# sehyun03/MulActSeg

Hardware: AMD Instinct MI355X
Metric: superpixels scored/sec (higher is better)
Workload: dtype f32; 1 GPU; acquisition-round: PixBal+ban-ignore scorer on resident logits, Cityscapes pool shape [4,20,1024,2048] per step; per rank K single-pass scans (class prior + region sums + histograms) of its shard, then exchange 1 (all-gather class sums) + device class weights (k_class_weight) + weighted finalize + ban + exchange 2 (all-gather scores) + replicated K4 (keys, radix sort, fair-counting budget walk) ov; nseg=2048, id_dtype=int64, regions_scored=679936, budget_clicks=11159, regions_selected=6688

## Files before the change

include/mulactseg_hip.h:

```cpp
#ifndef MULACTSEG_HIP_H
#define MULACTSEG_HIP_H

#include <stddef.h>
#include <stdint.h>

#ifdef __cplusplus
extern "C" {
#endif

#define MAS_ID_I64 0
#define MAS_ID_I32 1
#define MAS_ID_U16 2
#define MAS_MAP_U8 3

#define MAS_MAX_CLASSES 32

#define MAS_SCORE_FRAC_BITS 40
#define MAS_PROB_FRAC_BITS 23
#define MAS_LOSS_FRAC_BITS 32

#define MAS_ABI_VERSION 9
int mas_abi_version(void);
const char* mas_error_string(int code);

// ... 44 lines not shown
int mas_partial_loss_bwd(const float* z, const void* spx, int spx_dtype, const uint8_t* mask, const uint32_t* bits,
                         const uint64_t* gmax, const float* scale ,
                         int N, int C, int H, int W, int S, float invT, int flags, float* dz, void* stream);

int mas_partial_loss_fwd_lowres(const float* zq, int h, int w, const void* spx, int spx_dtype, const uint8_t* mask,
                                const uint32_t* bits, int N, int C, int H, int W, int S, float invT, int flags,
                                uint64_t* gmax , uint64_t* acc , void* stream);
int mas_partial_loss_bwd_lowres(const float* zq, int h, int w, const void* spx, int spx_dtype, const uint8_t* mask,
                                const uint32_t* bits, const uint64_t* gmax, const float* scale , int N, int C, int H, int W,
                                int S, float invT, int flags, int64_t* dzq_fix , void* stream);
#define MAS_GRAD_FRAC_BITS 44
int mas_fix_to_float(const int64_t* fix, int64_t n, int frac_bits, float* out, void* stream);

size_t mas_partial_loss_work_bytes(int N, int S, int C, int flags);
int mas_partial_loss_fwd_fused(const float* z, int h, int w, const void* spx, int spx_dtype, const uint8_t* mask, const uint8_t* targets,
                               int cols_stored, int cols_used, const uint32_t* bits, int N, int C, int H, int W, int S, float invT, int flags,
                               const float* weights, void* work, size_t work_bytes, float* losses, void* stream);
int mas_partial_loss_bwd_fused(const float* z, int h, int w, const void* spx, int spx_dtype, const uint8_t* mask, const uint32_t* bits,
                               const void* work, const float* grad, const float* weights, int N, int C, int H, int W, int S, float invT,
                               int flags, float* dz, int64_t* dzq_fix, void* stream);


int mas_region_keys(const float* score, const uint8_t* valid, const int32_t* img_rank, int64_t n_img, int S,
                    uint64_t* keys , void* stream);

size_t mas_select_workspace_bytes(int64_t n);

int mas_sort_keys_desc(const uint64_t* keys_in, int64_t n, uint64_t* keys_out, void* workspace, size_t ws_bytes,
                       void* stream);

int mas_budget_walk(const uint64_t* sorted_keys, int64_t n, const uint8_t* region_cost, const int32_t* img_of_rank,
                    int S, int64_t budget, int64_t max_out, int64_t* n_selected,
                    int32_t* sel_img, int32_t* sel_id, float* sel_score, void* workspace, size_t ws_bytes, void* stream);

int mas_region_reweight(float* score, const int32_t* dominant, int64_t n, int ban_class, const float* cls_w ,
                        void* stream);

int mas_dominant_hist(const int32_t* dominant, int64_t n, int C, uint64_t* counts , void* stream);

int mas_minmax_normalize(float* scores, int64_t n, uint32_t* scratch2, void* stream);


#define MAS_LABELS_BAD_VALUE 1

int mas_region_label_counts(const void* spx, int spx_dtype, const uint8_t* labels, int H, int W, int nseg, int num_classes, int trim_k,
                            int32_t* full , int32_t* trimmed , int32_t* status ,
                            void* stream);

int mas_region_multi_hot(const int32_t* full, const int32_t* trimmed, const uint8_t* listed, int nseg, int num_classes,
                         uint8_t* bits , int64_t* size , void* stream);

int mas_region_dominant(const int32_t* full, const uint8_t* listed, const int32_t* drawn , int nseg, int num_classes,
                        int generate_ignore, int32_t* choice , void* stream);

int mas_region_paint(const void* spx, int spx_dtype, const uint8_t* labels, int H, int W, int nseg, const int32_t* choice,
                     int generate_ignore, uint8_t* out , void* stream);

int mas_spx_max_onehot(const void* target, int target_dtype, const void* spx, int spx_dtype, int H, int W, int nseg, int num_classes,
                       int32_t* seg_max , int32_t* status , uint8_t* mask ,
                       uint8_t* rows , void* stream);


int mas_iou_counts(const int64_t* outputs, const int64_t* outputs_all, const int64_t* targets, int64_t n,
                   int num_classes, int64_t ignore_label, uint64_t* counts , void* stream);

int mas_logits_iou_counts(const float* z, const int64_t* targets, int B, int channels, int H, int W, int num_classes,
// ... 180 lines not shown
```

mulactseg_amd/_lib.py:

```python
import ctypes
import os

_HERE = os.path.dirname(os.path.abspath(__file__))
LIB_PATH = os.environ.get("MAS_LIB") or os.path.join(_HERE, "libmulactseg_hip.so")

ID_I64, ID_I32, ID_U16 = 0, 1, 2
MAP_U8 = 3
MAX_CLASSES = 32
LABELS_BAD_VALUE = 1
SCORE_FRAC, PROB_FRAC, LOSS_FRAC = 40, 23, 32
LOSS_CE, LOSS_GROUP, LOSS_GROUP_ONLY_MULTI, LOSS_DECOMP, LOSS_TCE = 1, 2, 4, 8, 16
ACC_WORDS = 8
GRAD_FRAC = 44
MS_MAX_SOURCES = 16

SK_DMA, SK_NOSPLIT = 1, 2
LOWRES_GENERIC = 1
ABI_VERSION = 9

_c = ctypes
_vp, _i, _f, _i64, _d = _c.c_void_p, _c.c_int, _c.c_float, _c.c_int64, _c.c_double


class SkOpts(ctypes.Structure):
    _fields_ = [("flags", _c.c_uint), ("spin_limit", _c.c_uint), ("stamps", _c.c_void_p)]


SIGNATURES = {
    "mas_abi_version": (_i, []),
    "mas_error_string": (_c.c_char_p, [_i]),
    "mas_class_prob_sum": (_i, [_vp, _i, _i, _i, _i, _f, _vp, _vp]),
    "mas_bvsb_region_accum": (_i, [_vp, _vp, _i, _vp, _i, _i, _i, _i, _i, _f, _vp, _vp, _vp]),
    "mas_region_finalize": (_i, [_vp, _vp, _i64, _i, _i, _vp, _vp, _vp, _vp, _vp]),
    "mas_region_keys": (_i, [_vp, _vp, _vp, _i64, _i, _vp, _vp]),
    "mas_select_workspace_bytes": (_c.c_size_t, [_i64]),
    "mas_sort_keys_desc": (_i, [_vp, _i64, _vp, _vp, _c.c_size_t, _vp]),
    "mas_budget_walk": (_i, [_vp, _i64, _vp, _vp, _i, _i64, _i64, _vp, _vp, _vp, _vp, _vp, _c.c_size_t, _vp]),
    "mas_region_reweight": (_i, [_vp, _vp, _i64, _i, _vp, _vp]),
    "mas_dominant_hist": (_i, [_vp, _i64, _i, _vp, _vp]),
    "mas_minmax_normalize": (_i, [_vp, _i64, _vp, _vp]),
    "mas_region_label_counts": (_i, [_vp, _i, _vp, _i, _i, _i, _i, _i, _vp, _vp, _vp, _vp]),
    "mas_region_multi_hot": (_i, [_vp, _vp, _vp, _i, _i, _vp, _vp, _vp]),
    "mas_region_dominant": (_i, [_vp, _vp, _vp, _i, _i, _i, _vp, _vp]),
    "mas_region_paint": (_i, [_vp, _i, _vp, _i, _i, _i, _vp, _i, _vp, _vp]),
    "mas_spx_max_onehot": (_i, [_vp, _i, _vp, _i, _i, _i, _i, _i, _vp, _vp, _vp, _vp, _vp]),
    "mas_iou_counts": (_i, [_vp, _vp, _vp, _i64, _i, _i64, _vp, _vp]),
    "mas_logits_iou_counts": (_i, [_vp, _vp, _i, _i, _i, _i, _i, _i64, _vp, _vp]),
    "mas_lowres_iou_counts": (_i, [_vp, _vp, _i, _i, _i, _i, _i, _i, _i, _i64, _vp, _vp]),
    "mas_single_pass_accum": (_i, [_vp, _vp, _i, _i, _i, _i, _i, _i, _f, _vp, _vp, _vp, _vp]),
    "mas_single_pass_accum_lowres": (_i, [_vp, _i, _i, _vp, _i, _i, _i, _i, _i, _i, _f, _vp, _vp, _vp, _vp]),
    "mas_single_pass_accum_lowres_opt": (_i, [_vp, _i, _i, _vp, _i, _i, _i, _i, _i, _i, _f, _vp, _vp, _vp, _c.c_uint, _vp]),
    "mas_class_weight": (_i, [_vp, _i, _i, _i64, _i, _i, _d, _vp, _vp, _vp, _vp]),
    "mas_region_finalize_weighted": (_i, [_vp, _vp, _i64, _i, _vp, _i, _vp, _vp, _vp, _vp, _vp]),
    "mas_stage2_gather_protos": (_i, [_vp, _i, _i, _i, _i, _i, _vp, _i, _vp, _vp]),
    "mas_stage2_assign": (_i, [_vp, _i, _i, _i, _i, _i, _vp, _vp, _i, _vp, _vp, _vp, _vp, _vp]),
    "mas_stage2_adjacency": (_i, [_vp, _i, _i, _i, _vp, _vp, _vp]),
    "mas_stage2_propagate": (_i, [_vp, _i, _i, _i, _i, _i, _vp, _i, _vp, _vp, _vp, _vp, _vp, _vp, _vp, _vp]),
    "mas_aspp_dw3_fwd": (_i, [_vp, _vp, _vp, _vp, _i, _i, _i, _i, _i, _i, _i, _vp, _vp, _vp, _vp]),
    "mas_aspp_dw3_bwd_x": (_i, [_vp, _vp, _vp, _vp, _vp, _vp, _i, _i, _i, _i, _i, _i, _i, _vp, _vp]),
    "mas_aspp_dw3_bwd_w": (_i, [_vp, _vp, _vp, _vp, _i, _i, _i, _i, _i, _i, _i, _vp, _vp, _vp, _vp]),
    "mas_train_augment": (_i, [_vp, _i, _i, _i, _i, _vp, _vp, _i, _vp, _vp, _i, _vp, _vp, _i, _i, _i, _i, _i, _i, _i, _vp, _vp, _vp,
                               _vp, _i, _i64, _vp, _i, _vp, _i, _i64, _vp, _i, _vp, _vp]),
    "mas_upsample_bilinear_fwd": (_i, [_vp, _i64, _i, _i, _i, _i, _vp, _vp]),
    "mas_upsample_bilinear_bwd": (_i, [_vp, _i64, _i, _i, _i, _i, _vp, _vp]),
    "mas_ms_ensemble": (_i, [_vp, _vp, _vp, _i, _i, _i, _i, _i, _vp, _vp, _vp]),
    "mas_naive_plbl": (_i, [_vp, _i, _i, _i, _i, _i, _i, _vp, _f, _vp, _vp]),
    "mas_ms_naive_plbl": (_i, [_vp, _vp, _i, _i, _i, _i, _vp, _i, _i64, _vp, _vp, _vp]),
    "mas_render_labels": (_i, [_vp, _i, _i, _i, _i, _vp, _i, _i, _vp, _i, _vp, _vp, _vp]),
    "mas_render_lowres_pred": (_i, [_vp, _i, _i, _i, _i, _i, _i, _vp, _i, _vp, _vp, _vp]),
    "mas_bn_workspace_bytes": (_i64, [_i, _i, _i]),
# ... 121 lines not shown
```

mulactseg_amd/active_selection/engine.py:

```python
import numpy as np
import torch


class ShardPlan:

    def __init__(self, n_img, batch_size, rank=0, world=1):
        self.n_img, self.batch_size, self.rank, self.world = n_img, batch_size, rank, world
        self.n_batches = (n_img + batch_size - 1) // batch_size
        per = (self.n_batches + world - 1) // world
        self.batch_lo = min(rank * per, self.n_batches)
        self.batch_hi = min((rank + 1) * per, self.n_batches)
        self.img_lo = min(self.batch_lo * batch_size, n_img)
        self.img_hi = min(self.batch_hi * batch_size, n_img)
        self.per_rank_imgs = per * batch_size
        self.batch_of = (np.arange(n_img) // batch_size).astype(np.int32)

    @property
    def local_indices(self):
        return list(range(self.img_lo, self.img_hi))

    @property
    def n_local(self):
        return self.img_hi - self.img_lo

# ... 16 lines not shown
        return local
    pad = torch.zeros((plan.per_rank_imgs,) + tuple(local.shape[1:]), dtype=local.dtype, device=local.device)
    pad[:plan.n_local] = local
    out = torch.empty((plan.world * plan.per_rank_imgs,) + tuple(local.shape[1:]), dtype=local.dtype, device=local.device)
    d.all_gather_into_tensor(out, pad)
    return out[:plan.n_img].contiguous()


def class_weight_from_sums(prob_sum, hw, batch_of, n_batches, coeff):
    prob_sum = np.ascontiguousarray(prob_sum).view(np.uint64)
    n_img, C = prob_sum.shape
    batch_of = np.asarray(batch_of)
    sums = np.zeros((n_batches, C), dtype=np.uint64)
    np.add.at(sums, batch_of, prob_sum)
    n_in = np.bincount(batch_of, minlength=n_batches)[:n_batches]
    live = n_in > 0
    terms = (sums[live].astype(np.float64) / np.float64(8388608.0)) / (n_in[live].astype(np.float64) * np.float64(hw))[:, None]
    acc = np.cumsum(terms, axis=0)[-1] if terms.shape[0] else np.zeros(C, dtype=np.float64)
    cum = acc / np.float64(n_batches)
    t = np.float64(coeff) * cum + np.float64(1.0)
    return cum, (np.float64(1.0) / (t * t)).astype(np.float32)


class HipBackend:
    name = "hip"

    def __init__(self, device):
        from .. import _lib, ops
        self.device = torch.device(device)
        if self.device.type != 'cuda':
            raise _lib.MulActSegHipError("HipBackend needs a ROCm device, got %s (no CPU path exists)" % device)
        _lib.load()
        self.ops = ops

    def inv_temperature(self, T):
        return self.ops.inv_temperature(T)

    def class_prob_sum(self, logits, invT, out):
        self.ops.class_prob_sum(logits, invT, out=out)

    def region_accum(self, logits, spx, cls_w, S, invT, score_sum, hist):
        self.ops.bvsb_region_accum(logits, spx, cls_w, S, invT, score_sum=score_sum, hist=hist)

    def finalize(self, score_sum, hist, ban_class, want_hist_i64=False):
        return self.ops.region_finalize(score_sum, hist, ban_class, want_hist_i64)

    def single_pass(self, logits, spx, S, invT, prob_sum, class_sum, hist):
        self.ops.single_pass_accum(logits, spx, S, invT, prob_sum=prob_sum, class_sum=class_sum, hist=hist)

    def single_pass_lowres(self, zq, size, spx, S, invT, prob_sum, class_sum, hist):
        self.ops.single_pass_accum_lowres(zq, size, spx, S, invT, prob_sum=prob_sum, class_sum=class_sum, hist=hist)

    def class_weight(self, prob_sum, hw, batch_size, n_batches, coeff):
        cum, w, w31 = self.ops.class_weight(prob_sum.contiguous(), hw, batch_size, n_batches, coeff)
        w._mas_w31 = w31
        return cum, w

    def finalize_weighted(self, class_sum, hist, cls_w, ban_class, want_hist_i64=False):
        w31 = None if cls_w is None else getattr(cls_w, '_mas_w31', None)
        if w31 is None:
            w = torch.ones(hist.shape[-1], dtype=torch.float32, device=hist.device) if cls_w is None else cls_w.detach().to(hist.device)
            w31 = (w.double() * 2147483648.0).floor().to(torch.int64).view(torch.int32)[::2].contiguous()
        return self.ops.region_finalize_weighted(class_sum, hist, w31, ban_class, want_hist_i64)

    def minmax_normalize_(self, scores):
        return self.ops.minmax_normalize_(scores)

    def region_reweight_(self, scores, dominant, ban_class, cls_w):
        return self.ops.region_reweight_(scores, dominant, ban_class, cls_w)

    def dominant_hist(self, dominant, C):
        return self.ops.dominant_hist(dominant, C)

    def select(self, scores, valid, img_rank, img_of_rank, region_cost, budget, max_out):
        keys = self.ops.region_keys(scores, valid, img_rank)
        skeys = self.ops.sort_keys_desc(keys)
        nsel, simg, sid, ssc = self.ops.budget_walk(skeys, region_cost, img_of_rank, scores.shape[1], budget, max_out)
        n = int(nsel.item())
        return n, simg[:n].cpu().numpy(), sid[:n].cpu().numpy(), ssc[:n].cpu().numpy()

    def local_head(self, plan, scores, valid, img_rank, max_out):
        lo, hi = plan.img_lo, plan.img_hi
        head = torch.zeros(max_out, dtype=torch.int64, device=scores.device)
        if hi > lo:
            keys = self.ops.region_keys(scores[lo:hi].contiguous(), None if valid is None else valid[lo:hi].contiguous(),
                                        img_rank[lo:hi].contiguous())
            m = min(keys.numel(), max_out)
            head[:m] = self.ops.sort_keys_desc(keys)[:m]
        return head

    def walk_heads(self, heads, region_cost, img_of_rank, S, budget, max_out):
        nsel, simg, sid, ssc = self.ops.budget_walk(self.ops.sort_keys_desc(heads), region_cost, img_of_rank, S, budget, max_out)
        n = int(nsel.item())
        return n, simg[:n].cpu().numpy(), sid[:n].cpu().numpy(), ssc[:n].cpu().numpy()

    def select_sharded(self, plan, scores, valid, img_rank, img_of_rank, region_cost, budget, max_out):
        head = self.local_head(plan, scores, valid, img_rank, max_out)
        merged = torch.empty(plan.world * max_out, dtype=torch.int64, device=scores.device)
        _dist().all_gather_into_tensor(merged, head)
        return self.walk_heads(merged, region_cost, img_of_rank, scores.shape[1], budget, max_out)


def default_backend(device):
    return HipBackend(device)


def select_regions(backend, plan, scores, valid, img_rank, img_of_rank, region_cost, budget, max_out):
    if plan.world > 1 and max_out is not None and _dist() is not None and hasattr(backend, 'select_sharded'):
        return backend.select_sharded(plan, scores, valid, img_rank, img_of_rank, region_cost, budget, max_out)
    return backend.select(scores, valid, img_rank, img_of_rank, region_cost, budget, max_out)


class AcquisitionRound:

    def __init__(self, n_img, n_channels, n_superpixels, batch_size, temperature, backend, rank=None, world=None,
                 single_pass=False):
        r, w = current_rank_world()
        self.plan = ShardPlan(n_img, batch_size, r if rank is None else rank, w if world is None else world)
        self.C, self.S = n_channels, n_superpixels
        self.backend = backend
        self.invT = backend.inv_temperature(temperature)
        self.single_pass = single_pass
        dev = backend.device
        nl = max(self.plan.n_local, 1)
# ... 90 lines not shown
```

mulactseg_amd/csrc/select.hip:

```cpp
#include <cstring>

#include <rocprim/device/device_radix_sort.hpp>
#include <rocprim/device/device_scan.hpp>

#include "common.h"

namespace {

constexpr int kThreads = 256;

__device__ __forceinline__ unsigned order_bits(float f) {
    const unsigned b = mas_f2u(f);
    return (b & 0x80000000u) ? ~b : (b | 0x80000000u);
}
__device__ __forceinline__ float unorder_bits(unsigned o) {
    return mas_u2f((o & 0x80000000u) ? (o & 0x7fffffffu) : ~o);
}

inline int id_bits_for(int S) {
    int b = 1;
    while ((1LL << b) < S) ++b;
    return b;
}

// ... 90 lines not shown
    }
    __syncthreads();
    if ((int)threadIdx.x < C && s_cnt[threadIdx.x]) atomicAdd(&counts[threadIdx.x], (mas_u64)s_cnt[threadIdx.x]);
}

__global__ __launch_bounds__(kThreads) void k_minmax_nonzero(const float* __restrict__ u, long long n, unsigned* __restrict__ mm) {
    unsigned lo = 0xffffffffu, hi = 0u;
    for (long long i = (long long)blockIdx.x * kThreads + threadIdx.x; i < n; i += (long long)gridDim.x * kThreads) {
        const float v = u[i];
        const unsigned o = order_bits(v);
        if (v != 0.0f) lo = o < lo ? o : lo;
        hi = o > hi ? o : hi;
    }
#pragma unroll
    for (int off = MAS_WAVE / 2; off > 0; off >>= 1) {
        const unsigned l2 = __shfl_down(lo, off, MAS_WAVE), h2 = __shfl_down(hi, off, MAS_WAVE);
        lo = l2 < lo ? l2 : lo;
        hi = h2 > hi ? h2 : hi;
    }
    if ((threadIdx.x & (MAS_WAVE - 1)) == 0) {
        atomicMin(&mm[0], lo);
        atomicMax(&mm[1], hi);
    }
}

__global__ void k_minmax_init(unsigned* mm) { mm[0] = 0xffffffffu; mm[1] = 0u; }

__global__ __launch_bounds__(kThreads) void k_minmax_apply(float* __restrict__ u, long long n, const unsigned* __restrict__ mm) {
    const long long i = (long long)blockIdx.x * kThreads + threadIdx.x;
    if (i >= n) return;
    const float mn = unorder_bits(mm[0]);
    const float mx = unorder_bits(mm[1]) - mn;
    u[i] = (u[i] - mn) / mx;
}

inline size_t align_up(size_t v) { return (v + 255) & ~(size_t)255; }

size_t sort_temp_bytes(long long n) {
    size_t bytes = 0;
    mas_u64* nul = nullptr;
    (void)rocprim::radix_sort_keys_desc(nullptr, bytes, nul, nul, (size_t)n, 0, 64, (hipStream_t)0);
    return bytes;
}
size_t scan_temp_bytes(long long n) {
    size_t bytes = 0;
    unsigned* nul = nullptr;
    (void)rocprim::inclusive_scan(nullptr, bytes, nul, nul, (size_t)n, rocprim::plus<unsigned>(), (hipStream_t)0);
    return bytes;
}

}

extern "C" size_t mas_select_workspace_bytes(int64_t n) {
    if (n <= 0) return 0;
    const size_t t = sort_temp_bytes(n), u = scan_temp_bytes(n);
    return align_up(t > u ? t : u) + 2 * align_up(sizeof(unsigned) * (size_t)n) + 256;
}

extern "C" int mas_region_keys(const float* score, const uint8_t* valid, const int32_t* img_rank, int64_t n_img, int S,
                               uint64_t* keys, void* stream) {
    if (!score || !img_rank || !keys) return MAS_ERR_NULL;
    if (n_img <= 0 || S <= 0) return MAS_ERR_SHAPE;
    const int b = id_bits_for(S);
    if (b > 24 || n_img > (1LL << (32 - b))) return MAS_ERR_RANGE;
    const long long n = (long long)n_img * S;
    const long long nblk = (n + kThreads - 1) / kThreads;
// ... 15 lines not shown
    return e == hipSuccess ? mas_launch_status() : (int)e;
}

extern "C" int mas_budget_walk(const uint64_t* sorted_keys, int64_t n, const uint8_t* region_cost, const int32_t* img_of_rank,
                               int S, int64_t budget, int64_t max_out, int64_t* n_selected, int32_t* sel_img, int32_t* sel_id,
                               float* sel_score, void* workspace, size_t ws_bytes, void* stream) {
    if (!sorted_keys || !img_of_rank || !n_selected || !sel_img || !sel_id || !sel_score || !workspace) return MAS_ERR_NULL;
    if (n <= 0 || S <= 0 || max_out <= 0 || budget < 0) return MAS_ERR_SHAPE;
    if (n > (1LL << 24)) return MAS_ERR_RANGE;
    if (ws_bytes < mas_select_workspace_bytes(n)) return MAS_ERR_WORKSPACE;
    hipStream_t st = static_cast<hipStream_t>(stream);
    const int b = id_bits_for(S);
    unsigned char* ws = static_cast<unsigned char*>(workspace);
    size_t temp = scan_temp_bytes(n);
    const size_t t = sort_temp_bytes(n);
    const size_t temp_region = align_up(t > temp ? t : temp);
    unsigned* cost = reinterpret_cast<unsigned*>(ws + temp_region);
    unsigned* prefix = reinterpret_cast<unsigned*>(ws + temp_region + align_up(sizeof(unsigned) * (size_t)n));
    const mas_u64* keys = reinterpret_cast<const mas_u64*>(sorted_keys);
    unsigned long long* nsel = reinterpret_cast<unsigned long long*>(n_selected);
    const long long nblk = (n + kThreads - 1) / kThreads;
    hipLaunchKernelGGL(k_set_u64, dim3(1), dim3(1), 0, st, nsel, (unsigned long long)n);
    hipLaunchKernelGGL(k_walk_cost, dim3((unsigned)nblk), dim3(kThreads), 0, st, keys, (long long)n, region_cost, img_of_rank, S, b, cost);
    hipError_t e = rocprim::inclusive_scan(ws, temp, cost, prefix, (size_t)n, rocprim::plus<unsigned>(), st);
    if (e != hipSuccess) return (int)e;
    hipLaunchKernelGGL(k_walk_find, dim3((unsigned)nblk), dim3(kThreads), 0, st, keys, prefix, (long long)n,
                       (unsigned long long)budget, nsel);
    const long long oblk = (max_out + kThreads - 1) / kThreads;
    hipLaunchKernelGGL(k_walk_emit, dim3((unsigned)oblk), dim3(kThreads), 0, st, keys, nsel, (long long)max_out, img_of_rank, b,
                       sel_img, sel_id, sel_score);
    return mas_launch_status();
}

extern "C" int mas_minmax_normalize(float* scores, int64_t n, uint32_t* scratch2, void* stream) {
    if (!scores || !scratch2) return MAS_ERR_NULL;
    if (n <= 0) return MAS_ERR_SHAPE;
    hipStream_t st = static_cast<hipStream_t>(stream);
    long long nblk = (n + kThreads - 1) / kThreads;
    hipLaunchKernelGGL(k_minmax_init, dim3(1), dim3(1), 0, st, scratch2);
    hipLaunchKernelGGL(k_minmax_nonzero, dim3((unsigned)(nblk > 1024 ? 1024 : nblk)), dim3(kThreads), 0, st, scores, (long long)n, scratch2);
    hipLaunchKernelGGL(k_minmax_apply, dim3((unsigned)nblk), dim3(kThreads), 0, st, scores, (long long)n, scratch2);
    return mas_launch_status();
}

extern "C" int mas_region_reweight(float* score, const int32_t* dominant, int64_t n, int ban_class, const float* cls_w, void* stream) {
    if (!score || !dominant) return MAS_ERR_NULL;
    if (n <= 0) return MAS_ERR_SHAPE;
    const long long nblk = (n + kThreads - 1) / kThreads;
    hipLaunchKernelGGL(k_region_reweight, dim3((unsigned)nblk), dim3(kThreads), 0, static_cast<hipStream_t>(stream), score, dominant,
                       (long long)n, ban_class, cls_w);
    return mas_launch_status();
}

extern "C" int mas_dominant_hist(const int32_t* dominant, int64_t n, int C, uint64_t* counts, void* stream) {
    if (!dominant || !counts) return MAS_ERR_NULL;
    if (n <= 0) return MAS_ERR_SHAPE;
    if (C < 1 || C > MAS_MAX_CLASSES) return MAS_ERR_CLASSES;
    long long nblk = (n + kThreads - 1) / kThreads;
    if (nblk > 1024) nblk = 1024;
    hipLaunchKernelGGL(k_dominant_hist, dim3((unsigned)nblk), dim3(kThreads), 0, static_cast<hipStream_t>(stream), dominant,
                       (long long)n, C, reinterpret_cast<mas_u64*>(counts));
    return mas_launch_status();
}
```

mulactseg_amd/ops.py:

```python
import ctypes
import os

import numpy as np
import torch

from . import _lib

_ID_CODES = {torch.int64: _lib.ID_I64, torch.int32: _lib.ID_I32, torch.uint16: _lib.ID_U16,
             torch.int16: _lib.ID_U16}


def inv_temperature(T):
    return float(np.float32(1.0) / np.float32(T))


def _stream(t):
    return torch.cuda.current_stream(t.device).cuda_stream


def _need(t, name, dtype=None):
    if not t.is_cuda:
        raise _lib.MulActSegHipError("%s must live on the GPU (no CPU path exists)" % name)
    if dtype is not None and t.dtype != dtype:
        raise TypeError("%s must be %s, got %s" % (name, dtype, t.dtype))
# ... 277 lines not shown
def sort_keys_desc(keys):
    _need(keys, "keys", torch.int64)
    n = keys.numel()
    lib = _lib.load()
    ws = torch.empty(lib.mas_select_workspace_bytes(n), dtype=torch.uint8, device=keys.device)
    out = torch.empty_like(keys)
    with torch.cuda.device(keys.device):
        _lib.check(lib.mas_sort_keys_desc(keys.data_ptr(), n, out.data_ptr(), ws.data_ptr(), ws.numel(), _stream(keys)),
                   "mas_sort_keys_desc")
    return out


def budget_walk(sorted_keys, region_cost, img_of_rank, S, budget, max_out=None):
    _need(sorted_keys, "sorted_keys", torch.int64)
    _need(img_of_rank, "img_of_rank", torch.int32)
    cost_bits = region_cost
    if cost_bits is not None:
        _need(cost_bits, "region_cost", torch.uint8)
    n = sorted_keys.numel()
    max_out = n if max_out is None else min(n, max_out)
    dev = sorted_keys.device
    lib = _lib.load()
    ws = torch.empty(lib.mas_select_workspace_bytes(n), dtype=torch.uint8, device=dev)
    nsel = torch.empty(1, dtype=torch.int64, device=dev)
    sel_img = torch.empty(max_out, dtype=torch.int32, device=dev)
    sel_id = torch.empty(max_out, dtype=torch.int32, device=dev)
    sel_score = torch.empty(max_out, dtype=torch.float32, device=dev)
    with torch.cuda.device(dev):
        _lib.check(lib.mas_budget_walk(sorted_keys.data_ptr(), n, cost_bits.data_ptr() if cost_bits is not None else None,
                                       img_of_rank.data_ptr(), S, int(budget), max_out, nsel.data_ptr(), sel_img.data_ptr(),
                                       sel_id.data_ptr(), sel_score.data_ptr(), ws.data_ptr(), ws.numel(), _stream(sorted_keys)),
                   "mas_budget_walk")
    return nsel, sel_img, sel_id, sel_score


def minmax_normalize_(scores):
    _need(scores, "scores", torch.float32)
    scratch = torch.empty(2, dtype=torch.int32, device=scores.device)
    with torch.cuda.device(scores.device):
        _lib.check(_lib.load().mas_minmax_normalize(scores.data_ptr(), scores.numel(), scratch.data_ptr(), _stream(scores)),
                   "mas_minmax_normalize")
    return scores


def iou_counts(outputs, outputs_all, targets, num_classes, ignore_label, counts=None):
    _need(targets, "targets", torch.int64)
    if outputs is not None:
        _need(outputs, "outputs", torch.int64)
    if outputs_all is not None:
        _need(outputs_all, "outputs_all", torch.int64)
    if counts is None:
        counts = torch.zeros(3 * num_classes + 3, dtype=torch.int64, device=targets.device)
    with torch.cuda.device(targets.device):
        _lib.check(_lib.load().mas_iou_counts(outputs.data_ptr() if outputs is not None else None,
                                              outputs_all.data_ptr() if outputs_all is not None else None,
                                              targets.data_ptr(), targets.numel(), num_classes, int(ignore_label),
                                              counts.data_ptr(), _stream(targets)), "mas_iou_counts")
    return counts


def logits_iou_counts(z, targets, num_classes, ignore_label, counts=None):
    _need(z, "logits", torch.float32)
    _need(targets, "targets", torch.int64)
    B, CH, H, W = z.shape
    if tuple(targets.shape) != (B, H, W):
        raise ValueError("targets %s do not match logits %s" % (tuple(targets.shape), tuple(z.shape)))
# ... 1871 lines not shown
```

Baseline: 55.93 million superpixels/s.

## Replace full radix sort with radix top-k prefix selection before budget walk

Adds a top-k selection path that histograms the high key bits, compacts only candidates above the k-th boundary, and refines with multi-level radix splits instead of radix-sorting all scored regions. For small k it ranks and walks the prefix in shared memory; otherwise it sorts only k keys. The selected results are packed into a single buffer copied to pinned host memory, replacing several separate device-to-host transfers. It adds many kernel launches and a fallback path when the prefix is insufficient for the budget.

```diff
diff --git a/include/mulactseg_hip.h b/include/mulactseg_hip.h
--- a/include/mulactseg_hip.h
+++ b/include/mulactseg_hip.h
@@ -100,6 +100,12 @@
 int mas_budget_walk(const uint64_t* sorted_keys, int64_t n, const uint8_t* region_cost, const int32_t* img_of_rank,
                     int S, int64_t budget, int64_t max_out, int64_t* n_selected,
                     int32_t* sel_img, int32_t* sel_id, float* sel_score, void* workspace, size_t ws_bytes, void* stream);
+
+size_t mas_select_prefix_workspace_bytes(int64_t n, int64_t k);
+
+int mas_select_prefix(const float* score, const uint8_t* valid, const int32_t* img_rank, const uint64_t* keys, int64_t n,
+                      int S, const uint8_t* region_cost, const int32_t* img_of_rank, int64_t budget, int64_t k,
+                      void* out, uint64_t* head, void* workspace, size_t ws_bytes, void* stream);
 
 int mas_region_reweight(float* score, const int32_t* dominant, int64_t n, int ban_class, const float* cls_w ,
                         void* stream);
diff --git a/mulactseg_amd/_lib.py b/mulactseg_amd/_lib.py
--- a/mulactseg_amd/_lib.py
+++ b/mulactseg_amd/_lib.py
@@ -36,6 +36,8 @@
     "mas_select_workspace_bytes": (_c.c_size_t, [_i64]),
     "mas_sort_keys_desc": (_i, [_vp, _i64, _vp, _vp, _c.c_size_t, _vp]),
     "mas_budget_walk": (_i, [_vp, _i64, _vp, _vp, _i, _i64, _i64, _vp, _vp, _vp, _vp, _vp, _c.c_size_t, _vp]),
+    "mas_select_prefix_workspace_bytes": (_c.c_size_t, [_i64, _i64]),
+    "mas_select_prefix": (_i, [_vp, _vp, _vp, _vp, _i64, _i, _vp, _vp, _i64, _i64, _vp, _vp, _vp, _c.c_size_t, _vp]),
     "mas_region_reweight": (_i, [_vp, _vp, _i64, _i, _vp, _vp]),
     "mas_dominant_hist": (_i, [_vp, _i64, _i, _vp, _vp]),
     "mas_minmax_normalize": (_i, [_vp, _i64, _vp, _vp]),
diff --git a/mulactseg_amd/active_selection/engine.py b/mulactseg_amd/active_selection/engine.py
--- a/mulactseg_amd/active_selection/engine.py
+++ b/mulactseg_amd/active_selection/engine.py
@@ -72,6 +72,7 @@
             raise _lib.MulActSegHipError("HipBackend needs a ROCm device, got %s (no CPU path exists)" % device)
         _lib.load()
         self.ops = ops
+        self._pinned = None
 
     def inv_temperature(self, T):
         return self.ops.inv_temperature(T)
@@ -112,7 +113,24 @@
     def dominant_hist(self, dominant, C):
         return self.ops.dominant_hist(dominant, C)
 
+    def _prefix_walk(self, max_out, S, budget, region_cost, img_of_rank, **src):
+        packed, _ = self.ops.select_prefix(max_out, S, region_cost=region_cost, img_of_rank=img_of_rank, budget=budget, **src)
+        if self._pinned is None or self._pinned.numel() < packed.numel():
+            self._pinned = torch.empty(2 * packed.numel(), dtype=torch.uint8, pin_memory=True)
+        host = self._pinned[:packed.numel()]
+        host.copy_(packed, non_blocking=True)
+        torch.cuda.current_stream(packed.device).synchronize()
+        n, status, simg, sid, ssc = self.ops.unpack_prefix(host.numpy())
+        if status:
+            return None
+        return n, simg[:n].copy(), sid[:n].copy(), ssc[:n].copy()
+
     def select(self, scores, valid, img_rank, img_of_rank, region_cost, budget, max_out):
+        if max_out is not None and max_out < scores.numel():
+            r = self._prefix_walk(max_out, scores.shape[1], budget, region_cost, img_of_rank, scores=scores, valid=valid,
+                                  img_rank=img_rank)
+            if r is not None:
+                return r
         keys = self.ops.region_keys(scores, valid, img_rank)
         skeys = self.ops.sort_keys_desc(keys)
         nsel, simg, sid, ssc = self.ops.budget_walk(skeys, region_cost, img_of_rank, scores.shape[1], budget, max_out)
@@ -121,6 +139,10 @@
 
     def local_head(self, plan, scores, valid, img_rank, max_out):
         lo, hi = plan.img_lo, plan.img_hi
+        if hi > lo and max_out < (hi - lo) * scores.shape[1]:
+            return self.ops.select_prefix(max_out, scores.shape[1], scores=scores[lo:hi].contiguous(),
+                                          valid=None if valid is None else valid[lo:hi].contiguous(),
+                                          img_rank=img_rank[lo:hi].contiguous(), walk=False, head=True)[1]
         head = torch.zeros(max_out, dtype=torch.int64, device=scores.device)
         if hi > lo:
             keys = self.ops.region_keys(scores[lo:hi].contiguous(), None if valid is None else valid[lo:hi].contiguous(),
@@ -130,6 +152,10 @@
         return head
 
     def walk_heads(self, heads, region_cost, img_of_rank, S, budget, max_out):
+        if max_out < heads.numel():
+            r = self._prefix_walk(max_out, S, budget, region_cost, img_of_rank, keys=heads)
+            if r is not None:
+                return r
         nsel, simg, sid, ssc = self.ops.budget_walk(self.ops.sort_keys_desc(heads), region_cost, img_of_rank, S, budget, max_out)
         n = int(nsel.item())
         return n, simg[:n].cpu().numpy(), sid[:n].cpu().numpy(), ssc[:n].cpu().numpy()
diff --git a/mulactseg_amd/csrc/select.hip b/mulactseg_amd/csrc/select.hip
--- a/mulactseg_amd/csrc/select.hip
+++ b/mulactseg_amd/csrc/select.hip
@@ -146,6 +146,386 @@
     const float mn = unorder_bits(mm[0]);
     const float mx = unorder_bits(mm[1]) - mn;
     u[i] = (u[i] - mn) / mx;
+}
+
+constexpr int kSelBits = 12;
+constexpr int kSelBins = 1 << kSelBits;
+constexpr int kSelShift0 = 64 - kSelBits;
+constexpr int kSelLds = 8192;
+constexpr int kFinThreads = 1024;
+constexpr int kSelChunk = 4 * kThreads;
+constexpr int kSelUnroll = 4;
+constexpr int kRankParts = 16;
+constexpr int kRankUnroll = 8;
+constexpr long long kSelWide = 1LL << 20;
+constexpr unsigned kSelSingle = 1u << 16;
+constexpr int kSelLevels = 4;
+
+enum { kMetaCand = 0, kMetaTop, kMetaNnz, kMetaKept, kMetaLevelCnt = 4 , kMetaState = 16,
+       kStAbove = 0, kStInBin, kStPrefixLo, kStPrefixHi, kStShift, kStBuf, kStWords, kMetaWords = kMetaState + kStWords * (kSelLevels + 1) };
+constexpr int kSelHdrWords = kSelBins * (kSelLevels + 1) + kMetaWords;
+
+struct SelLevel {
+    unsigned above, in_bin, shift, buf;
+    mas_u64 prefix;
+    __device__ static SelLevel load(const unsigned* meta, int l) {
+        const unsigned* w = meta + kMetaState + kStWords * l;
+        return SelLevel{w[kStAbove], w[kStInBin], w[kStShift], w[kStBuf], ((mas_u64)w[kStPrefixHi] << 32) | w[kStPrefixLo]};
+    }
+    __device__ void store(unsigned* meta, int l) const {
+        unsigned* w = meta + kMetaState + kStWords * l;
+        w[kStAbove] = above;
+        w[kStInBin] = in_bin;
+        w[kStShift] = shift;
+        w[kStBuf] = buf;
+        w[kStPrefixLo] = (unsigned)prefix;
+        w[kStPrefixHi] = (unsigned)(prefix >> 32);
+    }
+};
+
+constexpr size_t kOutHead = 16;
+
+struct ScoreKeys {
+    const float* score;
+    const unsigned char* valid;
+    const int* img_rank;
+    int S, id_bits;
+    __device__ __forceinline__ unsigned lo(long long i) const {
+        const long long img = i / S;
+        return ((unsigned)img_rank[img] << id_bits) | (unsigned)(i - img * S);
+    }
+    __device__ __forceinline__ bool top(long long i, unsigned& d) const {
+        if (valid && !valid[i]) return false;
+        const unsigned hi = order_bits(score[i]);
+        d = hi >> (32 - kSelBits);
+        return hi != 0 || lo(i) != 0;
+    }
+    __device__ __forceinline__ mas_u64 key(long long i) const {
+        return (valid && !valid[i]) ? 0 : (((mas_u64)order_bits(score[i]) << 32) | lo(i));
+    }
+};
+
+struct GivenKeys {
+    const mas_u64* keys;
+    __device__ __forceinline__ bool top(long long i, unsigned& d) const {
+        const mas_u64 k = keys[i];
+        d = (unsigned)(k >> kSelShift0);
+        return k != 0;
+    }
+    __device__ __forceinline__ mas_u64 key(long long i) const { return keys[i]; }
+};
+
+__global__ __launch_bounds__(kFinThreads) void k_sel_clear(unsigned* __restrict__ hdr, int words) {
+    for (int i = threadIdx.x; i < words; i += kFinThreads) hdr[i] = 0;
+}
+
+template <class Src>
+__global__ __launch_bounds__(kThreads) void k_sel_hist(Src src, long long n, unsigned* __restrict__ hist) {
+    __shared__ unsigned h[kSelBins];
+    for (int b = threadIdx.x; b < kSelBins; b += kThreads) h[b] = 0;
+    __syncthreads();
+    for (long long i = (long long)blockIdx.x * kThreads + threadIdx.x; i < n; i += (long long)gridDim.x * kThreads) {
+        unsigned d;
+        if (src.top(i, d)) atomicAdd(&h[d], 1u);
+    }
+    __syncthreads();
+    for (int b = threadIdx.x; b < kSelBins; b += kThreads)
+        if (h[b]) atomicAdd(&hist[b], h[b]);
+}
+
+template <int NT>
+__device__ void sel_boundary(const unsigned* h, unsigned need, unsigned* wsum, unsigned* res) {
+    constexpr int per = kSelBins / NT;
+    const int t = threadIdx.x, lane = t & (MAS_WAVE - 1), wave = t / MAS_WAVE;
+    unsigned own = 0;
+#pragma unroll
+    for (int j = 0; j < per; ++j) own += h[t * per + j];
+    unsigned s = own;
+#pragma unroll
+    for (int off = 1; off < MAS_WAVE; off <<= 1) {
+        const unsigned v = __shfl_down(s, off, MAS_WAVE);
+        if (lane + off < MAS_WAVE) s += v;
+    }
+    if (lane == 0) wsum[wave] = s;
+    __syncthreads();
+    for (int w = wave + 1; w < NT / MAS_WAVE; ++w) s += wsum[w];
+    if (t == 0) res[3] = s;
+    const unsigned above = s - own;
+    if (above < need && need <= s) {
+        unsigned run = above;
+        for (int j = per - 1; j >= 0; --j) {
+            const unsigned c = h[t * per + j];
+            if (run + c >= need) {
+                res[0] = (unsigned)(t * per + j);
+                res[1] = run;
+                res[2] = c;
+                break;
+            }
+            run += c;
+        }
+    }
+    __syncthreads();
+}
+
+template <class Src>
+__global__ __launch_bounds__(kThreads) void k_sel_compact(Src src, long long n, long long k, const unsigned* __restrict__ hist,
+                                                           unsigned* __restrict__ meta, mas_u64* __restrict__ top,
+                                                           mas_u64* __restrict__ cand) {
+    __shared__ unsigned h[kSelBins];
+    __shared__ unsigned wsum[kThreads / MAS_WAVE], res[4], cnt[2], base[2];
+    __shared__ mas_u64 stage[2][kSelChunk];
+    for (int b = threadIdx.x; b < kSelBins; b += kThreads) h[b] = hist[b];
+    if (threadIdx.x == 0) res[0] = res[1] = res[2] = 0;
+    __syncthreads();
+    sel_boundary<kThreads>(h, (unsigned)k, wsum, res);
+    const bool all = (unsigned long long)res[3] <= (unsigned long long)k;
+    const unsigned b1 = res[0];
+    if (blockIdx.x == 0 && threadIdx.x == 0) {
+        meta[kMetaNnz] = res[3];
+        SelLevel{all ? res[3] : res[1], all ? 0 : res[2], (unsigned)kSelShift0, 0, b1}.store(meta, 0);
+    }
+    for (long long c0 = (long long)blockIdx.x * kSelChunk; c0 < n; c0 += (long long)gridDim.x * kSelChunk) {
+        if (threadIdx.x < 2) cnt[threadIdx.x] = 0;
+        __syncthreads();
+#pragma unroll
+        for (int j = 0; j < kSelChunk / kThreads; ++j) {
+            const long long i = c0 + j * kThreads + threadIdx.x;
+            unsigned d;
+            if (i < n && src.top(i, d) && d >= b1) {
+                const int l = (all || d > b1) ? 0 : 1;
+                stage[l][atomicAdd(&cnt[l], 1u)] = src.key(i);
+            }
+        }
+        __syncthreads();
+        if (threadIdx.x < 2 && cnt[threadIdx.x])
+            base[threadIdx.x] = atomicAdd(&meta[threadIdx.x == 0 ? kMetaTop : kMetaCand], cnt[threadIdx.x]);
+        __syncthreads();
+        for (unsigned j = threadIdx.x; j < cnt[0]; j += kThreads) top[base[0] + j] = stage[0][j];
+        for (unsigned j = threadIdx.x; j < cnt[1]; j += kThreads) cand[base[1] + j] = stage[1][j];
+        __syncthreads();
+    }
+}
+
+__device__ __forceinline__ bool sel_level_active(const SelLevel& st, unsigned target) {
+    return st.in_bin > kSelSingle && (unsigned long long)st.above + st.in_bin > target && st.shift > 0;
+}
+
+__global__ __launch_bounds__(kThreads) void k_sel_level_hist(const mas_u64* __restrict__ cand, const mas_u64* __restrict__ cand2,
+                                                              const unsigned* __restrict__ meta, int l, unsigned target,
+                                                              unsigned* __restrict__ hist) {
+    const SelLevel st = SelLevel::load(meta, l);
+    if (!sel_level_active(st, target)) return;
+    __shared__ unsigned h[kSelBins];
+    const mas_u64* src = st.buf ? cand2 : cand;
+    const int sh = (int)st.shift - (st.shift < kSelBits ? (int)st.shift : kSelBits);
+    for (int b = threadIdx.x; b < kSelBins; b += kThreads) h[b] = 0;
+    __syncthreads();
+    for (unsigned i = blockIdx.x * kThreads + threadIdx.x; i < st.in_bin; i += gridDim.x * kThreads)
+        atomicAdd(&h[(unsigned)(src[i] >> sh) & (kSelBins - 1)], 1u);
+    __syncthreads();
+    for (int b = threadIdx.x; b < kSelBins; b += kThreads)
+        if (h[b]) atomicAdd(&hist[b], h[b]);
+}
+
+__global__ __launch_bounds__(kThreads) void k_sel_level_split(mas_u64* __restrict__ cand, mas_u64* __restrict__ cand2,
+                                                               unsigned* __restrict__ meta, int l, long long k, unsigned target,
+                                                               const unsigned* __restrict__ hist, mas_u64* __restrict__ top) {
+    const SelLevel st = SelLevel::load(meta, l);
+    if (!sel_level_active(st, target)) {
+        if (blockIdx.x == 0 && threadIdx.x == 0) st.store(meta, l + 1);
+        return;
+    }
+    __shared__ unsigned h[kSelBins];
+    __shared__ unsigned wsum[kThreads / MAS_WAVE], res[4], cnt[2], base[2];
+    __shared__ mas_u64 stage[2][kSelChunk];
+    const int d = st.shift < kSelBits ? (int)st.shift : kSelBits, sh = (int)st.shift - d;
+    for (int b = threadIdx.x; b < kSelBins; b += kThreads) h[b] = hist[b];
+    __syncthreads();
+    sel_boundary<kThreads>(h, (unsigned)(k - st.above), wsum, res);
+    const unsigned bb = res[0];
+    if (blockIdx.x == 0 && threadIdx.x == 0)
+        SelLevel{st.above + res[1], res[2], (unsigned)sh, st.buf ^ 1u, (st.prefix << d) | bb}.store(meta, l + 1);
+    const mas_u64* src = st.buf ? cand2 : cand;
+    mas_u64* dst = st.buf ? cand : cand2;
+    for (unsigned c0 = blockIdx.x * kSelChunk; c0 < st.in_bin; c0 += gridDim.x * kSelChunk) {
+        if (threadIdx.x < 2) cnt[threadIdx.x] = 0;
+        __syncthreads();
+#pragma unroll
+        for (int j = 0; j < kSelChunk / kThreads; ++j) {
+            const unsigned i = c0 + j * kThreads + threadIdx.x;
+            if (i < st.in_bin) {
+                const mas_u64 key = src[i];
+                const unsigned dg = (unsigned)(key >> sh) & (kSelBins - 1);
+                if (dg >= bb) {
+                    const int q = dg > bb ? 0 : 1;
+                    stage[q][atomicAdd(&cnt[q], 1u)] = key;
+                }
+            }
+        }
+        __syncthreads();
+        if (threadIdx.x < 2 && cnt[threadIdx.x]) base[threadIdx.x] = atomicAdd(&meta[kMetaLevelCnt + 2 * l + threadIdx.x], cnt[threadIdx.x]);
+        __syncthreads();
+        for (unsigned j = threadIdx.x; j < cnt[0]; j += kThreads) top[st.above + base[0] + j] = stage[0][j];
+        for (unsigned j = threadIdx.x; j < cnt[1]; j += kThreads) dst[base[1] + j] = stage[1][j];
+        __syncthreads();
+    }
+}
+
+__global__ __launch_bounds__(kFinThreads) void k_sel_refine(mas_u64* __restrict__ cand, mas_u64* __restrict__ cand2,
+                                                             unsigned* __restrict__ meta, int level, long long k, unsigned target,
+                                                             mas_u64* __restrict__ top) {
+    __shared__ unsigned h[kSelBins], wsum[kFinThreads / MAS_WAVE], res[4], cnt[2];
+    const int t = threadIdx.x;
+    const SelLevel st = SelLevel::load(meta, level);
+    unsigned above = st.above, in_bin = st.in_bin;
+    mas_u64 prefix = st.prefix;
+    int shift = (int)st.shift;
+    mas_u64* src = st.buf ? cand2 : cand;
+    mas_u64* dst = st.buf ? cand : cand2;
+    while ((unsigned long long)above + in_bin > target && shift > 0) {
+        const int d = shift < kSelBits ? shift : kSelBits, sh = shift - d;
+        for (int b = t; b < kSelBins; b += kFinThreads) h[b] = 0;
+        __syncthreads();
+        for (unsigned i0 = t; i0 < in_bin; i0 += kSelUnroll * kFinThreads) {
+            mas_u64 key[kSelUnroll];
+#pragma unroll
+            for (int q = 0; q < kSelUnroll; ++q) key[q] = i0 + q * kFinThreads < in_bin ? src[i0 + q * kFinThreads] : 0;
+#pragma unroll
+            for (int q = 0; q < kSelUnroll; ++q)
+                if (i0 + q * kFinThreads < in_bin) atomicAdd(&h[(unsigned)(key[q] >> sh) & (kSelBins - 1)], 1u);
+        }
+        __syncthreads();
+        sel_boundary<kFinThreads>(h, (unsigned)(k - above), wsum, res);
+        const unsigned bb = res[0];
+        if (t == 0) cnt[0] = cnt[1] = 0;
+        __syncthreads();
+        for (unsigned i0 = t; i0 < in_bin; i0 += kSelUnroll * kFinThreads) {
+            mas_u64 key[kSelUnroll];
+#pragma unroll
+            for (int q = 0; q < kSelUnroll; ++q) key[q] = i0 + q * kFinThreads < in_bin ? src[i0 + q * kFinThreads] : 0;
+#pragma unroll
+            for (int q = 0; q < kSelUnroll; ++q) {
+                if (i0 + q * kFinThreads >= in_bin) continue;
+                const unsigned dg = (unsigned)(key[q] >> sh) & (kSelBins - 1);
+                if (dg > bb) top[above + atomicAdd(&cnt[0], 1u)] = key[q];
+                else if (dg == bb) dst[atomicAdd(&cnt[1], 1u)] = key[q];
+            }
+        }
+        prefix = (prefix << d) | bb;
+        shift = sh;
+        above += res[1];
+        in_bin = res[2];
+        mas_u64* tmp = src;
+        src = dst;
+        dst = tmp;
+        __syncthreads();
+    }
+    unsigned kept;
+    if ((unsigned long long)above + in_bin <= target) {
+        for (unsigned i = t; i < in_bin; i += kFinThreads) top[above + i] = src[i];
+        kept = above + in_bin;
+    } else {
+        for (unsigned i = above + t; i < (unsigned)k; i += kFinThreads) top[i] = prefix;
+        kept = (unsigned)k;
+    }
+    for (unsigned i = kept + t; i < (unsigned)k; i += kFinThreads) top[i] = 0;
+    if (t == 0) meta[kMetaKept] = kept;
+}
+
+__global__ __launch_bounds__(kThreads) void k_sel_rank(const mas_u64* __restrict__ top, const unsigned* __restrict__ meta, long long k,
+                                                        const unsigned char* __restrict__ region_cost, const int* __restrict__ img_of_rank,
+                                                        int S, int id_bits, unsigned char* __restrict__ out,
+                                                        unsigned* __restrict__ cost_sorted, mas_u64* __restrict__ head) {
+    __shared__ mas_u64 s[kSelLds];
+    const unsigned m = meta[kMetaKept];
+    const unsigned e0 = blockIdx.x * (kThreads / kRankParts);
+    if (e0 >= m) return;
+    const int t = threadIdx.x;
+    for (unsigned j = t; j < m; j += kThreads) s[j] = top[j];
+    __syncthreads();
+    const unsigned e = e0 + t / kRankParts, p = t % kRankParts;
+    const mas_u64 x = e < m ? s[e] : 0;
+    unsigned r = 0;
+    if (e < m) {
+#pragma unroll kRankUnroll
+        for (unsigned j = p; j < m; j += kRankParts) {
+            const mas_u64 y = s[j];
+            r += (y > x) | ((y == x) & (j < e));
+        }
+    }
+#pragma unroll
+    for (int off = 1; off < kRankParts; off <<= 1) r += __shfl_xor(r, off, MAS_WAVE);
+    if (e >= m || p != 0 || r >= (unsigned long long)k) return;
+    if (head) head[r] = x;
+    if (out) {
+        const unsigned lo = (unsigned)x;
+        const int img = img_of_rank[lo >> id_bits];
+        int* oimg = reinterpret_cast<int*>(out + kOutHead);
+        oimg[r] = img;
+        oimg[k + r] = (int)(lo & ((1u << id_bits) - 1u));
+        reinterpret_cast<float*>(oimg + 2 * k)[r] = unorder_bits((unsigned)(x >> 32));
+        cost_sorted[r] = region_cost ? (unsigned)region_cost[(long long)img * S + (lo & ((1u << id_bits) - 1u))] : 1u;
+    }
+}
+
+__global__ __launch_bounds__(kFinThreads) void k_sel_walk(const unsigned* __restrict__ meta, long long k,
+                                                           const unsigned* __restrict__ cost_sorted, unsigned long long budget,
+                                                           unsigned char* __restrict__ out, mas_u64* __restrict__ head) {
+    __shared__ unsigned wsum[kFinThreads / MAS_WAVE], first;
+    const int t = threadIdx.x;
+    const unsigned m = meta[kMetaKept], nnz = meta[kMetaNnz];
+    const unsigned L = m < (unsigned)k ? m : (unsigned)k;
+    if (head)
+        for (unsigned i = L + t; i < (unsigned)k; i += kFinThreads) head[i] = 0;
+    if (!out) return;
+    constexpr int kIpt = kSelLds / kFinThreads;
+    unsigned cost[kIpt], own = 0;
+#pragma unroll
+    for (int j = 0; j < kIpt; ++j) {
+        const unsigned i = t * kIpt + j;
+        cost[j] = i < L ? cost_sorted[i] : 0;
+        own += cost[j];
+    }
+    if (t == 0) first = 0xffffffffu;
+    const int lane = t & (MAS_WAVE - 1), wave = t / MAS_WAVE;
+    unsigned incl = own;
+#pragma unroll
+    for (int off = 1; off < MAS_WAVE; off <<= 1) {
+        const unsigned v = __shfl_up(incl, off, MAS_WAVE);
+        if (lane >= off) incl += v;
+    }
+    if (lane == MAS_WAVE - 1) wsum[wave] = incl;
+    __syncthreads();
+    unsigned run = incl - own;
+    for (int w = 0; w < wave; ++w) run += wsum[w];
+    unsigned hit = 0xffffffffu;
+#pragma unroll
+    for (int j = kIpt - 1; j >= 0; --j) {
+        unsigned r = run;
+#pragma unroll
+        for (int q = 0; q <= j; ++q) r += cost[q];
+        if ((unsigned long long)r > budget && t * kIpt + j < L) hit = t * kIpt + j;
+    }
+    if (hit != 0xffffffffu) atomicMin(&first, hit);
+    __syncthreads();
+    const bool crossed = first != 0xffffffffu, resolved = crossed || L == nnz;
+    const unsigned n = crossed ? first + 1 : L;
+    long long* o64 = reinterpret_cast<long long*>(out);
+    int* oimg = reinterpret_cast<int*>(out + kOutHead);
+    if (t == 0) {
+        o64[0] = n;
+        o64[1] = resolved ? 0 : 1;
+    }
+    for (unsigned i = n + t; i < (unsigned)k; i += kFinThreads) {
+        oimg[i] = -1;
+        oimg[k + i] = -1;
+        reinterpret_cast<float*>(oimg + 2 * k)[i] = 0.0f;
+    }
+}
+
+__global__ void k_sel_status(const unsigned* __restrict__ meta, const unsigned* __restrict__ prefix, long long k,
+                             unsigned long long budget, long long* __restrict__ out) {
+    out[1] = ((unsigned long long)meta[kMetaNnz] > (unsigned long long)k && (unsigned long long)prefix[k - 1] <= budget) ? 1 : 0;
 }
 
 inline size_t align_up(size_t v) { return (v + 255) & ~(size_t)255; }
@@ -227,6 +607,114 @@
     return mas_launch_status();
 }
 
+namespace {
+struct PrefixWs {
+    size_t cand, cand2, top, cost, sorted, prefix, temp, total;
+    PrefixWs(long long n, long long k) {
+        cand = align_up(sizeof(unsigned) * kSelHdrWords);
+        cand2 = cand + align_up(sizeof(mas_u64) * (size_t)n);
+        top = cand2 + align_up(sizeof(mas_u64) * (size_t)n);
+        const long long cap = k <= kSelLds ? prefix_target(k) : k;
+        cost = top + align_up(sizeof(mas_u64) * (size_t)cap);
+        sorted = prefix = temp = cost;
+        total = cost + align_up(sizeof(unsigned) * (size_t)k);
+        if (k > kSelLds) {
+            sorted = cost + align_up(sizeof(unsigned) * (size_t)k);
+            prefix = sorted + align_up(sizeof(mas_u64) * (size_t)k);
+            temp = prefix + align_up(sizeof(unsigned) * (size_t)k);
+            const size_t t = sort_temp_bytes(k), u = scan_temp_bytes(k);
+            total = temp + align_up(t > u ? t : u);
+        }
+    }
+    static long long prefix_target(long long k) {
+        long long t = 64;
+        while (t < k) t <<= 1;
+        return t;
+    }
+};
+
+template <class Src>
+int select_prefix(Src src, long long n, long long k, const uint8_t* region_cost, const int32_t* img_of_rank, int S, int id_bits,
+                  int64_t budget, void* out, uint64_t* head, unsigned char* ws, hipStream_t st) {
+    const PrefixWs L(n, k);
+    unsigned* hist = reinterpret_cast<unsigned*>(ws);
+    unsigned* meta = hist + kSelBins * (kSelLevels + 1);
+    mas_u64* cand = reinterpret_cast<mas_u64*>(ws + L.cand);
+    mas_u64* cand2 = reinterpret_cast<mas_u64*>(ws + L.cand2);
+    mas_u64* top = reinterpret_cast<mas_u64*>(ws + L.top);
+    unsigned* cost = reinterpret_cast<unsigned*>(ws + L.cost);
+    mas_u64* head64 = reinterpret_cast<mas_u64*>(head);
+    unsigned char* out8 = static_cast<unsigned char*>(out);
+    long long nblk = (n + kSelChunk - 1) / kSelChunk;
+    if (nblk > 1024) nblk = 1024;
+    const unsigned long long ubudget = (unsigned long long)budget;
+    const long long target = k <= kSelLds ? PrefixWs::prefix_target(k) : k;
+    hipLaunchKernelGGL(k_sel_clear, dim3(1), dim3(kFinThreads), 0, st, hist, kSelHdrWords);
+    hipLaunchKernelGGL(k_sel_hist<Src>, dim3((unsigned)nblk), dim3(kThreads), 0, st, src, n, hist);
+    hipLaunchKernelGGL(k_sel_compact<Src>, dim3((unsigned)nblk), dim3(kThreads), 0, st, src, n, k, hist, meta, top, cand);
+    const bool wide = n >= kSelWide;
+    if (wide)
+        for (int l = 0; l < kSelLevels; ++l) {
+            unsigned* hl = hist + kSelBins * (l + 1);
+            hipLaunchKernelGGL(k_sel_level_hist, dim3((unsigned)nblk), dim3(kThreads), 0, st, cand, cand2, meta, l, (unsigned)target, hl);
+            hipLaunchKernelGGL(k_sel_level_split, dim3((unsigned)nblk), dim3(kThreads), 0, st, cand, cand2, meta, l, k, (unsigned)target, hl,
+                               top);
+        }
+    hipLaunchKernelGGL(k_sel_refine, dim3(1), dim3(kFinThreads), 0, st, cand, cand2, meta, wide ? kSelLevels : 0, k, (unsigned)target,
+                       top);
+    if (k <= kSelLds) {
+        const unsigned rblk = (unsigned)((target + kThreads / kRankParts - 1) / (kThreads / kRankParts));
+        hipLaunchKernelGGL(k_sel_rank, dim3(rblk), dim3(kThreads), 0, st, top, meta, k, region_cost, img_of_rank, S, id_bits, out8, cost,
+                           head64);
+        hipLaunchKernelGGL(k_sel_walk, dim3(1), dim3(kFinThreads), 0, st, meta, k, cost, ubudget, out8, head64);
+        return mas_launch_status();
+    }
+    mas_u64* sorted = head ? head64 : reinterpret_cast<mas_u64*>(ws + L.sorted);
+    size_t temp = sort_temp_bytes(k);
+    hipError_t e = rocprim::radix_sort_keys_desc(ws + L.temp, temp, top, sorted, (size_t)k, 0, 64, st);
+    if (e != hipSuccess) return (int)e;
+    if (!out) return mas_launch_status();
+    unsigned* prefix = reinterpret_cast<unsigned*>(ws + L.prefix);
+    unsigned long long* nsel = static_cast<unsigned long long*>(out);
+    int* oimg = reinterpret_cast<int*>(out8 + kOutHead);
+    const long long kblk = (k + kThreads - 1) / kThreads;
+    hipLaunchKernelGGL(k_set_u64, dim3(1), dim3(1), 0, st, nsel, (unsigned long long)k);
+    hipLaunchKernelGGL(k_walk_cost, dim3((unsigned)kblk), dim3(kThreads), 0, st, sorted, k, region_cost, img_of_rank, S, id_bits, cost);
+    temp = scan_temp_bytes(k);
+    e = rocprim::inclusive_scan(ws + L.temp, temp, cost, prefix, (size_t)k, rocprim::plus<unsigned>(), st);
+    if (e != hipSuccess) return (int)e;
+    hipLaunchKernelGGL(k_walk_find, dim3((unsigned)kblk), dim3(kThreads), 0, st, sorted, prefix, k, ubudget, nsel);
+    hipLaunchKernelGGL(k_walk_emit, dim3((unsigned)kblk), dim3(kThreads), 0, st, sorted, nsel, k, img_of_rank, id_bits, oimg, oimg + k,
+                       reinterpret_cast<float*>(oimg + 2 * k));
+    hipLaunchKernelGGL(k_sel_status, dim3(1), dim3(1), 0, st, meta, prefix, k, ubudget, static_cast<long long*>(out));
+    return mas_launch_status();
+}
+}
+
+extern "C" size_t mas_select_prefix_workspace_bytes(int64_t n, int64_t k) {
+    if (n <= 0 || k <= 0) return 0;
+    return PrefixWs(n, k < n ? k : n).total;
+}
+
+extern "C" int mas_select_prefix(const float* score, const uint8_t* valid, const int32_t* img_rank, const uint64_t* keys, int64_t n,
+                                 int S, const uint8_t* region_cost, const int32_t* img_of_rank, int64_t budget, int64_t k, void* out,
+                                 uint64_t* head, void* workspace, size_t ws_bytes, void* stream) {
+    if ((!score && !keys) || (score && (keys || !img_rank)) || (!out && !head) || (out && !img_of_rank) || !workspace)
+        return MAS_ERR_NULL;
+    if (n <= 0 || S <= 0 || k <= 0 || budget < 0 || (score && n % S)) return MAS_ERR_SHAPE;
+    if (k > n) k = n;
+    const int b = id_bits_for(S);
+    if (n > 0x7fffffffLL || b > 24 || (score && n / S > (1LL << (32 - b)))) return MAS_ERR_RANGE;
+    if (k > (1LL << 24)) return MAS_ERR_RANGE;
+    if (ws_bytes < mas_select_prefix_workspace_bytes(n, k)) return MAS_ERR_WORKSPACE;
+    hipStream_t st = static_cast<hipStream_t>(stream);
+    unsigned char* ws = static_cast<unsigned char*>(workspace);
+    if (score)
+        return select_prefix(ScoreKeys{score, valid, img_rank, S, b}, n, k, region_cost, img_of_rank, S, b, budget, out, head, ws, st);
+    return select_prefix(GivenKeys{reinterpret_cast<const mas_u64*>(keys)}, n, k, region_cost, img_of_rank, S, b, budget, out, head,
+                         ws, st);
+}
+
 extern "C" int mas_minmax_normalize(float* scores, int64_t n, uint32_t* scratch2, void* stream) {
     if (!scores || !scratch2) return MAS_ERR_NULL;
     if (n <= 0) return MAS_ERR_SHAPE;
diff --git a/mulactseg_amd/ops.py b/mulactseg_amd/ops.py
--- a/mulactseg_amd/ops.py
+++ b/mulactseg_amd/ops.py
@@ -333,6 +333,48 @@
                                        sel_id.data_ptr(), sel_score.data_ptr(), ws.data_ptr(), ws.numel(), _stream(sorted_keys)),
                    "mas_budget_walk")
     return nsel, sel_img, sel_id, sel_score
+
+
+def select_prefix(k, S, scores=None, valid=None, img_rank=None, keys=None, region_cost=None, img_of_rank=None, budget=0,
+                  walk=True, head=False):
+    if scores is not None:
+        _need(scores, "scores", torch.float32)
+        _need(img_rank, "img_rank", torch.int32)
+        n = scores.numel()
+        if scores.dim() != 2 or scores.shape[1] != S:
+            raise ValueError("scores must be [n_img, S]")
+        if valid is not None:
+            valid = _mask_u8(valid)
+            if tuple(valid.shape) != tuple(scores.shape):
+                raise ValueError("valid must be [n_img, S]")
+        src = scores
+    else:
+        _need(keys, "keys", torch.int64)
+        n = keys.numel()
+        src = keys
+    if region_cost is not None:
+        _need(region_cost, "region_cost", torch.uint8)
+    if walk:
+        _need(img_of_rank, "img_of_rank", torch.int32)
+    k = min(int(k), n)
+    dev = src.device
+    lib = _lib.load()
+    ws = torch.empty(lib.mas_select_prefix_workspace_bytes(n, k), dtype=torch.uint8, device=dev)
+    packed = torch.empty(16 + 12 * k, dtype=torch.uint8, device=dev) if walk else None
+    top = torch.empty(k, dtype=torch.int64, device=dev) if head else None
+    ptr = lambda t: None if t is None else t.data_ptr()
+    with torch.cuda.device(dev):
+        _lib.check(lib.mas_select_prefix(ptr(scores), ptr(valid), ptr(img_rank), ptr(keys), n, S, ptr(region_cost),
+                                         ptr(img_of_rank) if walk else None, int(budget), k, ptr(packed), ptr(top), ws.data_ptr(),
+                                         ws.numel(), _stream(src)), "mas_select_prefix")
+    return packed, top
+
+
+def unpack_prefix(buf):
+    k = (buf.size - 16) // 12
+    head = buf[:16].view(np.int64)
+    body = buf[16:16 + 12 * k]
+    return int(head[0]), int(head[1]), body[:4 * k].view(np.int32), body[4 * k:8 * k].view(np.int32), body[8 * k:].view(np.float32)
 
 
 def minmax_normalize_(scores):
```

Result: faster. 56.62 million superpixels/s (median of 6 runs) (+1.2%).
